# richox/orz

Hardware: AMD Instinct MI355X
Metric: orz -l1 encode throughput (enwik8-shaped text, 100 MB, one 16 MiB block in flight) (higher is better)
Workload: dtype u8

## Files before the change

### orz_amd/csrc/backend_hip.h

```cpp
#pragma once
#include <hip/hip_runtime.h>

#include <cxxabi.h>

#include <chrono>
#include <condition_variable>
#include <algorithm>
#include <atomic>
#include <cstring>
#include <map>
#include <mutex>
#include <rocprim/rocprim.hpp>
#include <stdexcept>
#include <string>
#include <type_traits>
#include <vector>

#include "orz_kernels.h"
#include "orz_parse.h"
#include "orz_symrank.h"

namespace orz {

#define ORZ_HIP_CHECK(expr)                                                                              \
// ... 527 lines not shown
        ORZ_HIP_CHECK(ce);
        hipGraphExec_t ex = nullptr;
        hipError_t e = hipGraphInstantiate(&ex, g, nullptr, nullptr, 0);
        (void)hipGraphDestroy(g);
        if (e != hipSuccess) throw std::runtime_error(std::string("hipGraphInstantiate: ") + hipGetErrorString(e));
        graph_exec_[key] = ex;
        ORZ_HIP_CHECK(hipGraphLaunch(ex, stream_));
    }
    void graph_capture_abort() {
        if (!capturing_) return;
        capturing_ = false;
        hipGraph_t g = nullptr;
        (void)hipStreamEndCapture(stream_, &g);
        stream_ = run_stream_;
        if (g) (void)hipGraphDestroy(g);
        (void)hipGetLastError();
    }
    void set_graphs(bool on) { graphs_ = on; }
    void clear_graphs() {
        for (auto& kv : graph_exec_) (void)hipGraphExecDestroy(kv.second);
        graph_exec_.clear();
    }
    void set_profile(bool on) { profile_ = on; nev_used_ = 0; nest_ = 0; }
    void begin_encode() { nev_used_ = 0; nest_ = 0; ev_used_ = 0; }
    bool profile() const { return profile_; }

    void symrank(uint16_t* srstate, const uint32_t* gsym, uint16_t* grank, const uint32_t* rstart, uint32_t nitems, uint32_t* flags,
                 uint16_t* backup, uint16_t* keep) {
        static_assert((512 * kSrWords * 2) % 8 == 0, "the tables are copied in 8-byte words");
        const uint32_t nw = 512 * kSrWords * 2 / 8;
        launch(nw, SymGuardBegin{reinterpret_cast<const uint64_t*>(srstate), reinterpret_cast<uint64_t*>(backup), nw, flags});
        Bracket br(*this, profile_ ? KernelNames::lib("orz_symrank_kernel (+ guard)") : 0);
        timed_begin(1);
        hipLaunchKernelGGL(orz_symrank_kernel, dim3(512), dim3(64), 0, stream_, srstate, gsym, grank, rstart, (const uint16_t*)nullptr,
                           (const uint32_t*)nullptr);
        ORZ_HIP_CHECK(hipGetLastError());
        timed_end(1);
        const char* inj = getenv("ORZ_SYMRANK_INJECT");
        const long inject = inj ? atol(inj) : -1;
        if (inject >= 0 && (uint32_t)inject < nitems) launch(1, SymInject{gsym, grank, (uint32_t)inject});
        launch(SymCheck::kThreads, SymCheck{gsym, grank, nitems, flags, nullptr});
        hipLaunchKernelGGL(orz_symrank_kernel, dim3(512), dim3(64), 0, stream_, srstate, gsym, grank, rstart, (const uint16_t*)backup,
                           (const uint32_t*)flags);
        ORZ_HIP_CHECK(hipGetLastError());
        launch(SymCheck::kThreads, SymCheck{gsym, grank, nitems, flags + 1, flags});
        static const bool verify = getenv("ORZ_SYMRANK_VERIFY") && atoi(getenv("ORZ_SYMRANK_VERIFY"));
        if (verify && keep) {
            launch(SymCompare::kThreads, SymKeep{grank, keep, nitems});
            hipLaunchKernelGGL(orz_symrank_kernel, dim3(512), dim3(64), 0, stream_, srstate, gsym, grank, rstart, (const uint16_t*)backup,
                               (const uint32_t*)nullptr);
            ORZ_HIP_CHECK(hipGetLastError());
            launch(SymCompare::kThreads, SymCompare{grank, keep, nitems, flags + 2});
        }
    }

   private:
    void* arena_take(size_t bytes) {
        if (!arena_on_) return nullptr;
        if (!arena_tried_) {
            arena_tried_ = true;
            const char* v = getenv("ORZ_ARENA_MB");
            const size_t mb = v ? (size_t)strtoull(v, nullptr, 10) : 0;
            if (mb) {
                (void)hipSetDevice(device_);
                void* p = nullptr;
                if (hipMalloc(&p, mb << 20) == hipSuccess) { arena_ = (char*)p; arena_bytes_ = mb << 20; }
                else (void)hipGetLastError();
            }
        }
        if (!arena_) return nullptr;
        const size_t align = bytes >= (1u << 20) ? (2u << 20) : 256;
        const size_t at = (arena_used_ + align - 1) / align * align;
        if (at + bytes > arena_bytes_) return nullptr;
        arena_used_ = at + bytes;
        arena_live_++;
        return arena_ + at;
    }
    char* arena_ = nullptr;
    size_t arena_bytes_ = 0, arena_used_ = 0, arena_live_ = 0;
    bool arena_tried_ = false, arena_on_ = false;
    int device_;
    bool lone_ = true, rank_prio_ = false;
// ... 25 lines not shown
```

### orz_amd/csrc/orz_capi.hip

```cpp
#include <cstdlib>
#include <cstring>
#include <map>
#include <memory>
#include <new>
#include <string>
#include <atomic>
#include <thread>
#include <vector>

#include "../../include/orz_hip.h"
#include "backend_hip.h"
#include "orz_decode_device.h"
#include "orz_decode_index.h"
#include "orz_decode_range.h"
#include "orz_decode_scatter.h"
#include "orz_host_decode.h"
#include "orz_planes.h"
#include "orz_decode_check.h"
#include "orz_stream.h"
#include "orz_fast_step.h"

namespace {
struct HwQueueDefault {
    HwQueueDefault() { setenv("GPU_MAX_HW_QUEUES", "16", 0); }
} g_hw_queue_default;


thread_local std::string g_err;
int fail(int code, const std::string& msg) {
    g_err = msg;
    return code;
}

orz::Cfg to_cfg(const orz_lzcfg* c) {
    return orz::Cfg{(int)c->match_depth, (int)c->lazy_match_depth1, (int)c->lazy_match_depth2};
}
// ... 30 lines not shown
    }
}

using Enc = orz::StreamEncoder<orz::HipBackend>;

bool mode_from_env() {
    const char* v = std::getenv("ORZ_MODE");
    return !(v && std::string(v) == "exact");
}

bool verify_decode_on() {
    const char* v = std::getenv("ORZ_VERIFY");
    return v && std::string(v) == "decode";
}
void verify_stream_decode(const uint8_t* src, size_t n, bool src_on_device, const uint8_t* out, size_t out_len) {
    std::vector<uint8_t> host;
    if (src_on_device && n) {
        host.resize(n);
        ORZ_HIP_CHECK(hipMemcpy(host.data(), src, n, hipMemcpyDeviceToHost));
        src = host.data();
    }
    orz::host::DecodeCheck chk;
    chk.feed_input(src, n);
    chk.feed_output(out, out_len);
    chk.finish();
}

unsigned window_for(const orz::HipBackend& be, const orz_lzcfg& c, unsigned asked) {
    if (asked) return asked;
    const size_t dmax = std::max(c.match_depth, std::max(c.lazy_match_depth1, c.lazy_match_depth2));
    return be.resident_parse_waves(orz::ParseLds::make((uint32_t)dmax, false).total);
}

}

struct orz_stream {
    std::unique_ptr<orz::HipBackend> be;
    std::unique_ptr<Enc> enc;
    orz_lzcfg cfg;
    unsigned seg, win;
    orz::ItemTrace trace;
    bool tracing = false;
    orz::FastTableCapture tables;
    bool fast = false;
    unsigned ftile = orz::kFastTile, frounds = orz::kFastRounds;
    unsigned unit = 0;
    double kernel_ms[4] = {0, 0, 0, 0};
    uint64_t kernel_n[4] = {0, 0, 0, 0};
    std::vector<orz::KernelRow> ktable;
    void rebuild() {
        std::unique_ptr<Enc> fresh;
        try {
            fresh.reset(new Enc(*be, to_cfg(&cfg), seg, fast ? 64 : window_for(*be, cfg, win), fast, ftile, frounds));
        } catch (const std::exception&) {
            if (!enc) throw;
            (void)hipGetLastError();
            enc.reset();
            be->clear_graphs();
            fresh.reset(new Enc(*be, to_cfg(&cfg), seg, fast ? 64 : window_for(*be, cfg, win), fast, ftile, frounds));
        }
        if (fast && unit && !getenv("ORZ_FAST_UNIT")) fresh->set_unit(unit);
        be->clear_graphs();
        enc = std::move(fresh);
        enc->trace = tracing ? &trace : nullptr;
        enc->tables = &tables;
    }
// ... 19 lines not shown
    std::unique_ptr<Enc> enc;
    orz_lzcfg cfg{0, 0, 0};
    unsigned seg, win;
    std::vector<uint8_t> framed;
    size_t framed_pos = 0;
    std::vector<size_t> chunk_end_spos;
    size_t next_chunk = 0;
    size_t expect_spos = 0;
    bool first_block = true;
    bool slid = false;
};

extern "C" {

const char* orz_last_error(void) { return g_err.c_str(); }
const char* orz_version(void) { return "orz_hip 0.1 (bitstream: richox/orz 1.6.1)"; }

int orz_device_count(void) {
    int n = 0;
    if (hipGetDeviceCount(&n) != hipSuccess) return 0;
    return n;
}

int orz_lzcfg_from_level(int level, orz_lzcfg* out) {
    if (!out) return fail(ORZ_EINVAL, "null cfg");
    switch (level) {
        case 0: *out = orz_lzcfg{5, 3, 2}; return ORZ_OK;
        case 1: *out = orz_lzcfg{15, 9, 6}; return ORZ_OK;
        case 2: *out = orz_lzcfg{45, 27, 18}; return ORZ_OK;
        default: return fail(ORZ_EINVAL, "invalid level");
    }
}

void orz_free(void* p) { std::free(p); }

static orz_stream* stream_new(int device, const orz_lzcfg* cfg, bool lone) {
    if (!cfg_ok(cfg)) { fail(ORZ_EINVAL, "bad LZCfg"); return nullptr; }
    try {
        if (device < 0 || device >= orz_device_count()) { fail(ORZ_ENODEV, "no such HIP device"); return nullptr; }
        std::unique_ptr<orz_stream> s(new orz_stream);
        s->be.reset(new orz::HipBackend(device, lone));
        s->be->enable_arena();
        s->cfg = *cfg;
        s->seg = env_u("ORZ_SEG", kDefaultSeg);
        s->win = env_u("ORZ_WIN", 0);
        s->fast = mode_from_env();
        s->ftile = env_u("ORZ_FAST_TILE", orz::kFastTile);
        s->frounds = env_u("ORZ_FAST_ROUNDS", orz::kFastRounds);
        s->be->set_graphs(env_u("ORZ_GRAPHS", 1) != 0);
        if (!lone) s->unit = orz::kNewMax;
        s->rebuild();
        return s.release();
    } catch (const std::exception& e) {
        fail(ORZ_ENODEV, e.what());
        return nullptr;
    }
}
orz_stream* orz_stream_new(int device, const orz_lzcfg* cfg) { return stream_new(device, cfg, true); }
void orz_stream_free(orz_stream* s) {
    if (!s) return;
    s->enc.reset();
    s->be.reset();
    delete s;
}
int orz_stream_set_tuning(orz_stream* s, unsigned seg_bytes, unsigned window_segs) {
    if (!s) return fail(ORZ_EINVAL, "null stream");
    try {
        s->reconfigure([&] {
            if (seg_bytes) s->seg = seg_bytes;
            if (window_segs) s->win = window_segs;
        });
        return ORZ_OK;
    } catch (const std::exception& e) {
        return fail(ORZ_EINVAL, e.what());
    }
}
int orz_stream_set_mode(orz_stream* s, int mode, unsigned tile_bytes, unsigned rounds) {
    if (!s || (mode != ORZ_MODE_EXACT && mode != ORZ_MODE_FAST)) return fail(ORZ_EINVAL, "bad mode");
    try {
        s->reconfigure([&] {
            s->fast = mode == ORZ_MODE_FAST;
            if (tile_bytes) s->ftile = tile_bytes;
            if (rounds) s->frounds = rounds;
        });
        return ORZ_OK;
    } catch (const std::exception& e) {
        return fail(ORZ_EINVAL, e.what());
    }
}
int orz_stream_set_profile(orz_stream* s, int on) {
    if (!s) return fail(ORZ_EINVAL, "null stream");
    s->be->set_profile(on != 0);
    return ORZ_OK;
}
int orz_stream_get_kernel_times(orz_stream* s, double* ms4, uint64_t* launches4) {
    if (!s || !ms4 || !launches4) return fail(ORZ_EINVAL, "null argument");
// ... 49 lines not shown
    } else {
        (void)hipGetLastError();
    }
    struct Disarm {
        orz::FastTableCapture& c;
        ~Disarm() { c.arm = -1; }
    } disarm{s->tables};
    struct ClearPatches {
        orz_stream* s;
        ~ClearPatches() { if (s->enc) s->enc->clear_item_patches(); }
    } clear_patches{s};
    const auto r = orz::encode_stream_device(*s->enc, be, (const uint8_t*)src, n, src_on_device != 0, d_dst, d_cap, pinned);
    if (stats) {
        float total = 0;
        ORZ_HIP_CHECK(hipEventElapsedTime(&total, ev.a, ev.b));
        const orz::EncodeStats& st = s->enc->stats;
        stats->blocks = st.blocks; stats->sweeps = st.sweeps; stats->seg_evals = st.seg_evals;
        stats->items = st.items; stats->chunks = st.chunks; stats->in_bytes = st.in_bytes;
        stats->out_bytes = r.len;
        stats->t_prep_s = st.t_prep; stats->t_parse_s = st.t_parse; stats->t_post_s = st.t_post;
        stats->parse_kernel_ms = be.collect_timed(&stats->parse_launches, s->kernel_ms, s->kernel_n);
        stats->total_ms = total;
        stats->host_syncs = st.host_syncs + be.take_host_syncs();
        if (be.profile()) s->ktable = be.collect_named();
    }
    return r;
}
int orz_stream_encode(orz_stream* s, const void* src, size_t n, int src_on_device, uint8_t** dst, size_t* dst_len,
                      orz_encode_stats* stats) {
    if (!s || !dst || !dst_len || (!src && n)) return fail(ORZ_EINVAL, "null argument");
    if (!s->enc) return fail(ORZ_ENOMEM, "the stream has no encoder (a reconfiguration ran out of device memory)");
    try {
        const auto r = stream_encode_device(s, src, n, src_on_device, nullptr, 0, stats);
        uint8_t* p = (uint8_t*)std::malloc(r.len ? r.len : 1);
        if (!p) return fail(ORZ_ENOMEM, "out of host memory");
        const hipError_t ce = hipMemcpy(p, r.data, r.len, hipMemcpyDeviceToHost);
        if (stats) stats->host_syncs += 1;
        if (ce != hipSuccess) { std::free(p); return fail(ORZ_ENODEV, hipGetErrorString(ce)); }
        if (verify_decode_on()) {
            try { verify_stream_decode((const uint8_t*)src, n, src_on_device != 0, p, r.len); } catch (...) { std::free(p); throw; }
        }
        *dst_len = r.len;
        *dst = p;
        return ORZ_OK;
    } catch (const std::bad_alloc&) {
        return fail(ORZ_ENOMEM, "out of host memory");
    } catch (const std::exception& e) {
        return fail(ORZ_ENODEV, e.what());
    }
}
size_t orz_stream_bound(size_t n) { return orz::stream_bound(n); }
int orz_stream_encode_to_device(orz_stream* s, const void* src, size_t n, int src_on_device, uint8_t* d_dst, size_t d_cap,
                                size_t* dst_len, orz_encode_stats* stats) {
    if (!s || !d_dst || !dst_len || (!src && n)) return fail(ORZ_EINVAL, "null argument");
    if (!s->enc) return fail(ORZ_ENOMEM, "the stream has no encoder (a reconfiguration ran out of device memory)");
    try {
        const auto r = stream_encode_device(s, src, n, src_on_device, d_dst, d_cap, stats);
        if (verify_decode_on()) {
            std::vector<uint8_t> host(r.len);
            ORZ_HIP_CHECK(hipMemcpy(host.data(), r.data, r.len, hipMemcpyDeviceToHost));
            verify_stream_decode((const uint8_t*)src, n, src_on_device != 0, host.data(), host.size());
        }
        *dst_len = r.len;
        return ORZ_OK;
    } catch (const std::bad_alloc&) {
        return fail(ORZ_ENOMEM, "out of host memory");
    } catch (const std::exception& e) {
        const std::string msg = e.what();
        return fail(msg.find("output buffer is too small") != std::string::npos ? ORZ_ENOMEM : ORZ_ENODEV, msg);
    }
}

int orz_stream_set_item_trace(orz_stream* s, int on) {
// ... 985 lines not shown
```

### orz_amd/csrc/orz_symrank.h

```cpp
#pragma once
#include "orz_kernels.h"

namespace orz {

#if defined(__HIPCC__)

constexpr uint32_t kSrGroup = 32;
constexpr uint32_t kSrPad = 448;
constexpr uint32_t kSrValOff = 0;
constexpr uint32_t kSrIdxOff = 896;
constexpr uint32_t kSrSnapOff = 1792;
constexpr uint32_t kSrLdsBytes = kSrSnapOff + kSrGroup * 128;

#define ORZ_SRL_WB_1 "s_waitcnt lgkmcnt(1)\n\tds_write_b16 %[aw], %[n]\n\t"
#define ORZ_SRL_WB_0 "s_nop 0\n\t"
#define ORZ_SRL_ITEM(P, J2, SNAP, PREV)                                                                                  \
    "ds_write_b16 %[l2], %[x] offset:" SNAP "\n\t"                                                                       \
    "v_readlane_b32 %[si], %[x], " J2 "\n\t"                                                                             \
    "s_cmpk_ge_u32 %[qw], 0x1860\n\t"                         \
    ORZ_SRL_WB_##PREV                                                                                                    \
    "v_mov_b32 %[vi], %[si]\n\t"                                                                                         \
    "s_cbranch_scc1 " P "30f\n\t"                                                                                        \
    P "31:\n\t"                                                                                                          \
    "s_add_u32 %[qw], %[qw], 16\n\t"                                                                                     \
    "s_add_u32 %[qa], %[qa], %[si]\n\t"                                                                                  \
    "s_sub_u32 %[qa], %[qa], %[qc]\n\t"                                                                                  \
    "s_cmp_ge_u32 %[qa], %[qw]\n\t"                                                                                      \
    "v_lshrrev_b32 %[t], 4, %[vi]\n\t"                                                                                   \
    "v_lshrrev_b32 %[h], 1, %[vi]\n\t"                                                                                   \
    "v_sub_u32 %[t], %[vi], %[t]\n\t"                                                                                    \
    "s_cbranch_scc1 " P "40f\n\t"                                                                                        \
    P "41:\n\t"                                                                                                          \
    "v_sub_u32_e64 %[t], %[t], %[q]\n\t"                                                                                 \
    "v_cmp_eq_u32_e64 %[m1], %[x], %[vi]\n\t"                                                                            \
    "v_max3_i32 %[nx], %[t], %[h], 0\n\t"                                   \
    "v_add_u32 %[y], %[vi], %[nx]\n\t"                                                                                   \
    "v_cmp_eq_u32_e64 %[m3], %[x], %[nx]\n\t"                                                                            \
    "v_lshrrev_b32 %[y], 1, %[y]\n\t"                            \
    "v_cndmask_b32_e64 %[rr], %[nx], %[y], %[m01]\n\t"                    \
    "v_cmp_eq_u32_e32 vcc, %[x], %[y]\n\t"                                                                               \
    "v_cndmask_b32_e64 %[rw], %[y], %[vi], %[m01]\n\t"                      \
    "v_lshl_add_u32 %[ar], %[rr], 1, %[base]\n\t"                                                                        \
    "v_cndmask_b32_e64 %[x], %[x], %[y], %[m3]\n\t"                                                   \
    "ds_read_u16 %[n], %[ar]\n\t"                                                                                        \
    "v_cndmask_b32_e32 %[x], %[x], %[vi], vcc\n\t"             \
    "v_lshl_add_u32 %[aw], %[rw], 1, %[base]\n\t"                                                                        \
    "v_cndmask_b32_e64 %[x], %[x], %[nx], %[m1]\n\t"
#define ORZ_SRL_WBS_1 "s_waitcnt lgkmcnt(1)\n\tds_write_b16 %[aw], %[n]\n\t"
#define ORZ_SRL_WBS_0 "s_nop 1\n\t"
#define ORZ_SRL_ITEM_S(J2, SNAP, PREV)                                                                                   \
    "ds_write_b16 %[l2], %[x] offset:" SNAP "\n\t"                                                                       \
    "v_readlane_b32 %[si], %[x], " J2 "\n\t"                                                                             \
    ORZ_SRL_WBS_##PREV                                                                                                   \
    "v_mov_b32 %[vi], %[si]\n\t"                                                                                         \
    "v_mad_i32_i24 %[t], %[vi], 15, %[c15]\n\t"  \
    "v_lshrrev_b32 %[h], 1, %[vi]\n\t"                                                                                   \
    "v_cmp_eq_u32_e64 %[m1], %[x], %[vi]\n\t"                                                                            \
    "v_ashrrev_i32 %[t], 4, %[t]\n\t"                                                                                    \
    "v_max3_i32 %[nx], %[t], %[h], 0\n\t"                                                                                \
    "v_add_u32 %[y], %[vi], %[nx]\n\t"                                                                                   \
    "v_cmp_eq_u32_e64 %[m3], %[x], %[nx]\n\t"                                                                            \
    "v_lshrrev_b32 %[y], 1, %[y]\n\t"                                                                                    \
    "v_cndmask_b32_e64 %[rr], %[nx], %[y], %[m01]\n\t"                                                                   \
    "v_cmp_eq_u32_e32 vcc, %[x], %[y]\n\t"                                                                               \
    "v_cndmask_b32_e64 %[rw], %[y], %[vi], %[m01]\n\t"                                                                   \
    "v_lshl_add_u32 %[ar], %[rr], 1, %[base]\n\t"                                                                        \
    "v_cndmask_b32_e64 %[x], %[x], %[y], %[m3]\n\t"                                                                      \
    "ds_read_u16 %[n], %[ar]\n\t"                                                                                        \
    "v_cndmask_b32_e32 %[x], %[x], %[vi], vcc\n\t"                                                                       \
    "v_lshl_add_u32 %[aw], %[rw], 1, %[base]\n\t"                                                                        \
    "v_cndmask_b32_e64 %[x], %[x], %[nx], %[m1]\n\t"
#define ORZ_SRL_SIDE(P)                                                                                                  \
    P "30:\n\t"                                                             \
    "s_lshr_b32 %[s0], %[qw], 4\n\t"                                                                                     \
    "s_mul_i32 %[s1], %[s0], %[qc]\n\t"                                                                                  \
    "s_add_u32 %[s1], %[s1], %[qa]\n\t"                                                                                  \
    "s_mul_i32 %[s0], %[s0], 9\n\t"                                                                                      \
    "s_mul_hi_u32 %[s0], %[s0], 0xcccccccd\n\t"                                                                          \
    "s_lshr_b32 %[s0], %[s0], 3\n\t"                                                                                     \
    "s_mul_i32 %[s1], %[s1], 9\n\t"                                                                                      \
    "s_mul_hi_u32 %[s1], %[s1], 0xcccccccd\n\t"                                                                          \
    "s_lshr_b32 %[s1], %[s1], 3\n\t"                                                                                     \
    "s_lshl_b32 %[qw], %[s0], 4\n\t"                                                                                     \
    "s_mul_i32 %[s0], %[s0], %[qc]\n\t"                                                                                  \
    "s_sub_u32 %[qa], %[s1], %[s0]\n\t"                                                                                  \
    "s_branch " P "31b\n\t"                                                                                              \
    P "40:\n\t"                                                \
    "s_cmp_lt_i32 %[qa], 0\n\t"                                                                                          \
    "s_cbranch_scc1 " P "42f\n\t"                                                                                        \
    "s_sub_u32 %[qa], %[qa], %[qw]\n\t"                                                                                  \
    "s_add_u32 %[q], %[q], 1\n\t"                                                                                        \
    "s_add_u32 %[qc], %[qc], 16\n\t"                                                                                     \
    "s_branch " P "43f\n\t"                                                                                              \
    P "42:\n\t"                                                                                                          \
    "s_add_u32 %[qa], %[qa], %[qw]\n\t"                                                                                  \
    "s_sub_u32 %[q], %[q], 1\n\t"                                                                                        \
    "s_sub_u32 %[qc], %[qc], 16\n\t"                                                                                     \
    P "43:\n\t"                                                                                                          \
    "s_cmp_ge_u32 %[qa], %[qw]\n\t"                                                                                      \
    "s_cbranch_scc1 " P "40b\n\t"                                                                                        \
    "s_branch " P "41b\n\t"

// ... 35 lines not shown
    ORZ_SRL_SIDE("101") \
    ORZ_SRL_SIDE("102") \
    ORZ_SRL_SIDE("103") \
    ORZ_SRL_SIDE("104") \
    ORZ_SRL_SIDE("105") \
    ORZ_SRL_SIDE("106") \
    ORZ_SRL_SIDE("107") \
    ORZ_SRL_SIDE("108") \
    ORZ_SRL_SIDE("109") \
    ORZ_SRL_SIDE("110") \
    ORZ_SRL_SIDE("111") \
    ORZ_SRL_SIDE("112") \
    ORZ_SRL_SIDE("113") \
    ORZ_SRL_SIDE("114") \
    ORZ_SRL_SIDE("115") \
    ORZ_SRL_SIDE("116") \
    ORZ_SRL_SIDE("117") \
    ORZ_SRL_SIDE("118") \
    ORZ_SRL_SIDE("119") \
    ORZ_SRL_SIDE("120") \
    ORZ_SRL_SIDE("121") \
    ORZ_SRL_SIDE("122") \
    ORZ_SRL_SIDE("123") \
    ORZ_SRL_SIDE("124") \
    ORZ_SRL_SIDE("125") \
    ORZ_SRL_SIDE("126") \
    ORZ_SRL_SIDE("127") \
    ORZ_SRL_SIDE("128") \
    ORZ_SRL_SIDE("129") \
    ORZ_SRL_SIDE("130") \
    ORZ_SRL_SIDE("131") \
    "9:\n\t"

#define ORZ_SRL_GROUP_S \
    ORZ_SRL_ITEM_S("0", "0", 0) \
    ORZ_SRL_ITEM_S("2", "128", 1) \
    ORZ_SRL_ITEM_S("4", "256", 1) \
    ORZ_SRL_ITEM_S("6", "384", 1) \
    ORZ_SRL_ITEM_S("8", "512", 1) \
    ORZ_SRL_ITEM_S("10", "640", 1) \
    ORZ_SRL_ITEM_S("12", "768", 1) \
    ORZ_SRL_ITEM_S("14", "896", 1) \
    ORZ_SRL_ITEM_S("16", "1024", 1) \
    ORZ_SRL_ITEM_S("18", "1152", 1) \
    ORZ_SRL_ITEM_S("20", "1280", 1) \
    ORZ_SRL_ITEM_S("22", "1408", 1) \
    ORZ_SRL_ITEM_S("24", "1536", 1) \
    ORZ_SRL_ITEM_S("26", "1664", 1) \
    ORZ_SRL_ITEM_S("28", "1792", 1) \
    ORZ_SRL_ITEM_S("30", "1920", 1) \
    ORZ_SRL_ITEM_S("32", "2048", 1) \
    ORZ_SRL_ITEM_S("34", "2176", 1) \
    ORZ_SRL_ITEM_S("36", "2304", 1) \
    ORZ_SRL_ITEM_S("38", "2432", 1) \
    ORZ_SRL_ITEM_S("40", "2560", 1) \
    ORZ_SRL_ITEM_S("42", "2688", 1) \
    ORZ_SRL_ITEM_S("44", "2816", 1) \
    ORZ_SRL_ITEM_S("46", "2944", 1) \
    ORZ_SRL_ITEM_S("48", "3072", 1) \
    ORZ_SRL_ITEM_S("50", "3200", 1) \
    ORZ_SRL_ITEM_S("52", "3328", 1) \
    ORZ_SRL_ITEM_S("54", "3456", 1) \
    ORZ_SRL_ITEM_S("56", "3584", 1) \
    ORZ_SRL_ITEM_S("58", "3712", 1) \
    ORZ_SRL_ITEM_S("60", "3840", 1) \
    ORZ_SRL_ITEM_S("62", "3968", 1)

__global__ __launch_bounds__(64) void orz_symrank_kernel(uint16_t* srstate, const uint32_t* gsym, uint16_t* grank,
                                                         const uint32_t* rstart, const uint16_t* state_in, const uint32_t* only_if) {
    __shared__ __attribute__((aligned(16))) uint16_t lds[kSrLdsBytes / 2];
    uint16_t* const val = lds + kSrValOff / 2;
    uint16_t* const idx = lds + kSrIdxOff / 2;
    const uint32_t c = blockIdx.x, lane = threadIdx.x;
    if (only_if && *only_if == 0) return;
    const uint32_t a = rstart[c], e = rstart[c + 1];
    if (a >= e) return;
    __builtin_amdgcn_s_setprio(3);
    uint16_t* state = srstate + (size_t)c * kSrWords;
    const uint16_t* sin = state_in ? state_in + (size_t)c * kSrWords : state;
    const uint32_t base = (uint32_t)(uintptr_t)lds;
    auto slot_of = [&](uint32_t sym) -> uint32_t { return base + kSrIdxOff + 2 * sym; };
    auto sym_of = [&](uint32_t slot) -> uint32_t { return (slot - base - kSrIdxOff) >> 1; };
    typedef __attribute__((address_space(3))) uint16_t lds_u16;
    auto at = [&](uint32_t slot) -> lds_u16& { return *reinterpret_cast<lds_u16*>((uintptr_t)slot); };
    for (uint32_t i = lane; i < kSrPad; i += 64) {
        val[i] = (uint16_t)slot_of(i < kSyms ? sin[i] : i);
        idx[i] = i < kSyms ? sin[kSyms + i] : (uint16_t)i;
    }
    uint32_t cnt = __builtin_amdgcn_readfirstlane((int)(sin[2 * kSyms] | ((uint32_t)sin[2 * kSyms + 1] << 16)));
    uint32_t sum = __builtin_amdgcn_readfirstlane((int)(sin[2 * kSyms + 2] | ((uint32_t)sin[2 * kSyms + 3] << 16)));
    __syncthreads();
    bool idx_ok = true;
    auto rebuild_idx = [&]() {
        uint32_t s[7];
#pragma unroll
        for (uint32_t m = 0; m < 7; m++) s[m] = val[lane + 64 * m];
#pragma unroll
        for (uint32_t m = 0; m < 7; m++) at(s[m]) = (uint16_t)(lane + 64 * m);
    };
    auto load_pairs = [&](uint32_t j0) -> uint32_t {
        return j0 + kSrGroup <= e ? gsym[j0 + (lane >> 1)] : 0u;
    };
    auto out_rank = [&](uint32_t ri, uint32_t ru) -> uint16_t { return (uint16_t)(ri == ru ? kSyms - 1 : ri - (ri > ru)); };
    const uint32_t l2 = base + kSrSnapOff + 2 * lane;
    const uint32_t* const snap_pair = reinterpret_cast<const uint32_t*>(lds + kSrSnapOff / 2 + (lane & 31) * 66);
    const uint64_t m01 = 1;
    uint32_t j = a;
    while (j < e) {
        if (cnt >= 192 && e - j >= kSrGroup) {
            uint32_t q = (uint32_t)__builtin_amdgcn_readfirstlane((int)((sum >> 4) / cnt));
            uint32_t pairs = load_pairs(j);
            do {
                uint32_t s[7];
#pragma unroll
                for (uint32_t m = 0; m < 7; m++) s[m] = val[lane + 64 * m];
#pragma unroll
                for (uint32_t m = 0; m < 7; m++) at(s[m]) = (uint16_t)(lane + 64 * m);
                const uint32_t symslot = slot_of((lane & 1) ? pairs >> 16 : pairs & 0xffff);
                const int x0 = (int)at(symslot);
                pairs = load_pairs(j + kSrGroup);
                q = (uint32_t)__builtin_amdgcn_readfirstlane((int)q);
                uint32_t si;
                uint64_t m1, m3;
                int x, vi, t, h, nx, y, rr, rw, ar, aw, n;
                bool done = false;
                if (cnt >= 327 && q < 32) {
                    x = x0;
                    asm volatile("s_waitcnt lgkmcnt(0)\n\t"
                                 ORZ_SRL_GROUP_S
                                 "s_waitcnt lgkmcnt(0)\n\tds_write_b16 %[aw], %[n]\n\t"
                                 "v_lshl_add_u32 %[ar], %[x], 1, %[base]\n\tds_write_b16 %[ar], %[sym]\n\t"
                                 : [x] "+v"(x), [si] "=&s"(si), [m1] "=&s"(m1), [m3] "=&s"(m3), [vi] "=&v"(vi), [t] "=&v"(t), [h] "=&v"(h),
                                   [nx] "=&v"(nx), [y] "=&v"(y), [rr] "=&v"(rr), [rw] "=&v"(rw), [ar] "=&v"(ar), [aw] "=&v"(aw), [n] "=&v"(n)
                                 : [l2] "v"(l2), [base] "s"(base), [sym] "v"(symslot), [m01] "s"(m01), [c15] "s"(15 - (int)(q << 4))
                                 : "vcc", "memory");
                    const uint32_t two = *snap_pair;
                    uint32_t ps = lane < kSrGroup ? two & 0xffff : 0;
                    ps += (uint32_t)__builtin_amdgcn_update_dpp(0, (int)ps, 0x111, 0xf, 0xf, true);
                    ps += (uint32_t)__builtin_amdgcn_update_dpp(0, (int)ps, 0x112, 0xf, 0xf, true);
                    ps += (uint32_t)__builtin_amdgcn_update_dpp(0, (int)ps, 0x114, 0xf, 0xf, true);
                    ps += (uint32_t)__builtin_amdgcn_update_dpp(0, (int)ps, 0x118, 0xf, 0xf, true);
                    ps += (uint32_t)__builtin_amdgcn_update_dpp(0, (int)ps, 0x142, 0xa, 0xf, true);
                    const uint32_t r = kSyms + 1 - cnt;
                    const uint32_t pr = r > 0 && r < kSrGroup ? (uint32_t)__builtin_amdgcn_readlane((int)ps, (int)((r - 1) & 31)) : 0u;
                    const uint32_t scaled = (sum + pr) * 9 / 10;
                    const bool after = lane >= r;
                    const uint32_t cnt_k = after ? (kSyms + 1) * 9 / 10 + (lane - r) + 1 : cnt + lane + 1;
                    const uint32_t sum_k = after ? scaled + (ps - pr) : sum + ps;
                    const uint32_t lo = (q << 4) * cnt_k;
                    const bool ok = sum_k >= lo && sum_k - lo < (cnt_k << 4);
                    if (__ballot(lane < kSrGroup && !ok) == 0) {
                        if (lane < kSrGroup) grank[j + lane] = out_rank(two & 0xffff, two >> 16);
                        cnt = (uint32_t)__builtin_amdgcn_readlane((int)cnt_k, 31);
                        sum = (uint32_t)__builtin_amdgcn_readlane((int)sum_k, 31);
                        done = true;
                    } else {
#pragma unroll
                        for (uint32_t m = 0; m < 7; m++) val[lane + 64 * m] = (uint16_t)s[m];
                    }
                }
                if (!done) {
                    uint32_t s0, s1;
                    uint32_t qw = (uint32_t)__builtin_amdgcn_readfirstlane((int)(cnt << 4));
                    uint32_t qc = (uint32_t)__builtin_amdgcn_readfirstlane((int)(q << 4));
                    uint32_t qa = (uint32_t)__builtin_amdgcn_readfirstlane((int)(sum - q * qw));
                    x = x0;
                    asm volatile("s_waitcnt lgkmcnt(0)\n\t"
                                 ORZ_SRL_GROUP
                                 "s_waitcnt lgkmcnt(0)\n\tds_write_b16 %[aw], %[n]\n\t"
                                 "v_lshl_add_u32 %[ar], %[x], 1, %[base]\n\tds_write_b16 %[ar], %[sym]\n\t"
                                 : [x] "+v"(x), [qw] "+s"(qw), [qa] "+s"(qa), [qc] "+s"(qc), [q] "+s"(q), [si] "=&s"(si), [s0] "=&s"(s0),
                                   [s1] "=&s"(s1), [m1] "=&s"(m1), [m3] "=&s"(m3), [vi] "=&v"(vi), [t] "=&v"(t), [h] "=&v"(h), [nx] "=&v"(nx),
                                   [y] "=&v"(y), [rr] "=&v"(rr), [rw] "=&v"(rw), [ar] "=&v"(ar), [aw] "=&v"(aw), [n] "=&v"(n)
                                 : [l2] "v"(l2), [base] "s"(base), [sym] "v"(symslot), [m01] "s"(m01)
                                 : "scc", "vcc", "memory");
                    cnt = qw >> 4;
                    sum = qa + q * qw;
                    const uint32_t two = *snap_pair;
                    if (lane < kSrGroup) grank[j + lane] = out_rank(two & 0xffff, two >> 16);
                }
                j += kSrGroup;
            } while (e - j >= kSrGroup);
            idx_ok = false;
            continue;
        }
        if (!idx_ok) { rebuild_idx(); idx_ok = true; }
        const uint32_t g = __builtin_amdgcn_readfirstlane((int)gsym[j]);
        const uint32_t v = g & 0xffff, vun = g >> 16;
        const uint32_t i = idx[v], iu = idx[vun];
        if (cnt > kSyms) {
            cnt = cnt * 9 / 10;
            sum = sum * 9 / 10;
        }
        cnt += 1;
        sum += i;
        const uint32_t dec = ((i >> 4) + (((sum >> 4) / cnt) & 0xffff)) & 0xffff, half = i >> 1;
        uint32_t nx = i > dec ? i - dec : 0;
        nx = nx > half ? nx : half;
        const uint32_t y = (i + nx) >> 1;
        const uint32_t nv1 = val[y], nv2 = val[nx];
        val[y] = (uint16_t)nv2; at(nv2) = (uint16_t)y;
        val[i] = (uint16_t)nv1; at(nv1) = (uint16_t)i;
        val[nx] = (uint16_t)slot_of(v); idx[v] = (uint16_t)nx;
        if (lane == 0) grank[j] = out_rank(i, iu);
        j += 1;
    }
    if (!idx_ok) rebuild_idx();
    __syncthreads();
    for (uint32_t i = lane; i < kSyms; i += 64) { state[i] = (uint16_t)sym_of(val[i]); state[kSyms + i] = idx[i]; }
    if (lane == 0) {
        state[2 * kSyms] = (uint16_t)cnt;
        state[2 * kSyms + 1] = (uint16_t)(cnt >> 16);
        state[2 * kSyms + 2] = (uint16_t)sum;
        state[2 * kSyms + 3] = (uint16_t)(sum >> 16);
    }
}

#endif

}
```

Baseline: 495.6.

## Split symrank into producer and LDS-update helper waves; pool pinned result buffers

The symrank kernel now launches two waves per block. Wave 0 computes the rank chain and publishes snapshots, while wave 1 applies the LDS swap writes in sub-batches, synchronised by s_barrier and a control word in LDS. The intent is to take the serial read-modify-write LDS traffic off the critical wave. Separately, encode results of 1 MiB or more are copied into pooled pinned host buffers with an async copy, avoiding the cost of staging through pageable memory. The risks are barrier overhead per sub-batch, subtle ordering bugs in the hand-written asm protocol, and pooled buffers outliving their stream handles.

```diff
diff --git a/orz_amd/csrc/backend_hip.h b/orz_amd/csrc/backend_hip.h
--- a/orz_amd/csrc/backend_hip.h
+++ b/orz_amd/csrc/backend_hip.h
@@ -583,7 +583,7 @@
         launch(nw, SymGuardBegin{reinterpret_cast<const uint64_t*>(srstate), reinterpret_cast<uint64_t*>(backup), nw, flags});
         Bracket br(*this, profile_ ? KernelNames::lib("orz_symrank_kernel (+ guard)") : 0);
         timed_begin(1);
-        hipLaunchKernelGGL(orz_symrank_kernel, dim3(512), dim3(64), 0, stream_, srstate, gsym, grank, rstart, (const uint16_t*)nullptr,
+        hipLaunchKernelGGL(orz_symrank_kernel, dim3(512), dim3(kSrThreads), 0, stream_, srstate, gsym, grank, rstart, (const uint16_t*)nullptr,
                            (const uint32_t*)nullptr);
         ORZ_HIP_CHECK(hipGetLastError());
         timed_end(1);
@@ -591,14 +591,14 @@
         const long inject = inj ? atol(inj) : -1;
         if (inject >= 0 && (uint32_t)inject < nitems) launch(1, SymInject{gsym, grank, (uint32_t)inject});
         launch(SymCheck::kThreads, SymCheck{gsym, grank, nitems, flags, nullptr});
-        hipLaunchKernelGGL(orz_symrank_kernel, dim3(512), dim3(64), 0, stream_, srstate, gsym, grank, rstart, (const uint16_t*)backup,
+        hipLaunchKernelGGL(orz_symrank_kernel, dim3(512), dim3(kSrThreads), 0, stream_, srstate, gsym, grank, rstart, (const uint16_t*)backup,
                            (const uint32_t*)flags);
         ORZ_HIP_CHECK(hipGetLastError());
         launch(SymCheck::kThreads, SymCheck{gsym, grank, nitems, flags + 1, flags});
         static const bool verify = getenv("ORZ_SYMRANK_VERIFY") && atoi(getenv("ORZ_SYMRANK_VERIFY"));
         if (verify && keep) {
             launch(SymCompare::kThreads, SymKeep{grank, keep, nitems});
-            hipLaunchKernelGGL(orz_symrank_kernel, dim3(512), dim3(64), 0, stream_, srstate, gsym, grank, rstart, (const uint16_t*)backup,
+            hipLaunchKernelGGL(orz_symrank_kernel, dim3(512), dim3(kSrThreads), 0, stream_, srstate, gsym, grank, rstart, (const uint16_t*)backup,
                                (const uint32_t*)nullptr);
             ORZ_HIP_CHECK(hipGetLastError());
             launch(SymCompare::kThreads, SymCompare{grank, keep, nitems, flags + 2});
diff --git a/orz_amd/csrc/orz_capi.hip b/orz_amd/csrc/orz_capi.hip
--- a/orz_amd/csrc/orz_capi.hip
+++ b/orz_amd/csrc/orz_capi.hip
@@ -2,6 +2,7 @@
 #include <cstring>
 #include <map>
 #include <memory>
+#include <mutex>
 #include <new>
 #include <string>
 #include <atomic>
@@ -98,6 +99,77 @@
     return be.resident_parse_waves(orz::ParseLds::make((uint32_t)dmax, false).total);
 }
 
+}
+
+namespace {
+constexpr size_t kPoolMin = size_t(1) << 20;
+constexpr size_t kPoolIdleMax = 2;
+struct ResultPool {
+    std::mutex mu;
+    std::map<void*, size_t> out;
+    std::vector<std::pair<void*, size_t>> idle;
+    size_t handles = 0;
+    static size_t capacity_for(size_t n) {
+        size_t c = kPoolMin;
+        while (c < n) c <<= 1;
+        return c;
+    }
+    void* take(size_t n) {
+        const size_t cap = capacity_for(n);
+        {
+            std::lock_guard<std::mutex> g(mu);
+            size_t best = idle.size();
+            for (size_t i = 0; i < idle.size(); i++)
+                if (idle[i].second >= cap && (best == idle.size() || idle[i].second < idle[best].second)) best = i;
+            if (best < idle.size()) {
+                void* p = idle[best].first;
+                out[p] = idle[best].second;
+                idle.erase(idle.begin() + (long)best);
+                return p;
+            }
+        }
+        void* p = nullptr;
+        if (hipHostMalloc(&p, cap, hipHostMallocPortable) != hipSuccess || !p) {
+            (void)hipGetLastError();
+            return nullptr;
+        }
+        std::lock_guard<std::mutex> g(mu);
+        out[p] = cap;
+        return p;
+    }
+    bool give(void* p) {
+        size_t cap = 0;
+        {
+            std::lock_guard<std::mutex> g(mu);
+            auto it = out.find(p);
+            if (it == out.end()) return false;
+            cap = it->second;
+            out.erase(it);
+            if (handles > 0 && idle.size() < kPoolIdleMax) {
+                idle.emplace_back(p, cap);
+                return true;
+            }
+        }
+        (void)hipHostFree(p);
+        return true;
+    }
+    void handle_born() {
+        std::lock_guard<std::mutex> g(mu);
+        handles++;
+    }
+    void handle_gone() {
+        std::vector<std::pair<void*, size_t>> drop;
+        {
+            std::lock_guard<std::mutex> g(mu);
+            if (handles > 0 && --handles == 0) drop.swap(idle);
+        }
+        for (auto& b : drop) (void)hipHostFree(b.first);
+    }
+};
+ResultPool& result_pool() {
+    static ResultPool* const pool = new ResultPool;
+    return *pool;
+}
 }
 
 struct orz_stream {
@@ -183,7 +255,10 @@
     }
 }
 
-void orz_free(void* p) { std::free(p); }
+void orz_free(void* p) {
+    if (!p) return;
+    if (!result_pool().give(p)) std::free(p);
+}
 
 static orz_stream* stream_new(int device, const orz_lzcfg* cfg, bool lone) {
     if (!cfg_ok(cfg)) { fail(ORZ_EINVAL, "bad LZCfg"); return nullptr; }
@@ -201,6 +276,7 @@
         s->be->set_graphs(env_u("ORZ_GRAPHS", 1) != 0);
         if (!lone) s->unit = orz::kNewMax;
         s->rebuild();
+        result_pool().handle_born();
         return s.release();
     } catch (const std::exception& e) {
         fail(ORZ_ENODEV, e.what());
@@ -213,6 +289,7 @@
     s->enc.reset();
     s->be.reset();
     delete s;
+    result_pool().handle_gone();
 }
 int orz_stream_set_tuning(orz_stream* s, unsigned seg_bytes, unsigned window_segs) {
     if (!s) return fail(ORZ_EINVAL, "null stream");
@@ -328,13 +405,15 @@
     if (!s->enc) return fail(ORZ_ENOMEM, "the stream has no encoder (a reconfiguration ran out of device memory)");
     try {
         const auto r = stream_encode_device(s, src, n, src_on_device, nullptr, 0, stats);
-        uint8_t* p = (uint8_t*)std::malloc(r.len ? r.len : 1);
+        uint8_t* p = r.len >= kPoolMin ? (uint8_t*)result_pool().take(r.len) : nullptr;
+        if (!p) p = (uint8_t*)std::malloc(r.len ? r.len : 1);
         if (!p) return fail(ORZ_ENOMEM, "out of host memory");
-        const hipError_t ce = hipMemcpy(p, r.data, r.len, hipMemcpyDeviceToHost);
+        hipError_t ce = hipMemcpyAsync(p, r.data, r.len, hipMemcpyDeviceToHost, s->be->stream());
+        if (ce == hipSuccess) ce = hipStreamSynchronize(s->be->stream());
         if (stats) stats->host_syncs += 1;
-        if (ce != hipSuccess) { std::free(p); return fail(ORZ_ENODEV, hipGetErrorString(ce)); }
+        if (ce != hipSuccess) { orz_free(p); return fail(ORZ_ENODEV, hipGetErrorString(ce)); }
         if (verify_decode_on()) {
-            try { verify_stream_decode((const uint8_t*)src, n, src_on_device != 0, p, r.len); } catch (...) { std::free(p); throw; }
+            try { verify_stream_decode((const uint8_t*)src, n, src_on_device != 0, p, r.len); } catch (...) { orz_free(p); throw; }
         }
         *dst_len = r.len;
         *dst = p;
diff --git a/orz_amd/csrc/orz_symrank.h b/orz_amd/csrc/orz_symrank.h
--- a/orz_amd/csrc/orz_symrank.h
+++ b/orz_amd/csrc/orz_symrank.h
@@ -10,7 +10,15 @@
 constexpr uint32_t kSrValOff = 0;
 constexpr uint32_t kSrIdxOff = 896;
 constexpr uint32_t kSrSnapOff = 1792;
-constexpr uint32_t kSrLdsBytes = kSrSnapOff + kSrGroup * 128;
+constexpr uint32_t kSrCtlOff = kSrSnapOff + kSrGroup * 128;
+constexpr uint32_t kSrLdsBytes = kSrCtlOff + 16;
+constexpr uint32_t kSrThreads = 128;
+#ifndef ORZ_SR_SUB
+#define ORZ_SR_SUB 8
+#endif
+constexpr uint32_t kSrSub = ORZ_SR_SUB;
+static_assert(kSrSub == 4 || kSrSub == 8, "a sub-batch is 4 or 8 items");
+constexpr uint32_t kSrCtlExit = 0;
 
 #define ORZ_SRL_WB_1 "s_waitcnt lgkmcnt(1)\n\tds_write_b16 %[aw], %[n]\n\t"
 #define ORZ_SRL_WB_0 "s_nop 0\n\t"
@@ -44,30 +52,6 @@
     "v_cndmask_b32_e64 %[x], %[x], %[y], %[m3]\n\t"                                                   \
     "ds_read_u16 %[n], %[ar]\n\t"                                                                                        \
     "v_cndmask_b32_e32 %[x], %[x], %[vi], vcc\n\t"             \
-    "v_lshl_add_u32 %[aw], %[rw], 1, %[base]\n\t"                                                                        \
-    "v_cndmask_b32_e64 %[x], %[x], %[nx], %[m1]\n\t"
-#define ORZ_SRL_WBS_1 "s_waitcnt lgkmcnt(1)\n\tds_write_b16 %[aw], %[n]\n\t"
-#define ORZ_SRL_WBS_0 "s_nop 1\n\t"
-#define ORZ_SRL_ITEM_S(J2, SNAP, PREV)                                                                                   \
-    "ds_write_b16 %[l2], %[x] offset:" SNAP "\n\t"                                                                       \
-    "v_readlane_b32 %[si], %[x], " J2 "\n\t"                                                                             \
-    ORZ_SRL_WBS_##PREV                                                                                                   \
-    "v_mov_b32 %[vi], %[si]\n\t"                                                                                         \
-    "v_mad_i32_i24 %[t], %[vi], 15, %[c15]\n\t"  \
-    "v_lshrrev_b32 %[h], 1, %[vi]\n\t"                                                                                   \
-    "v_cmp_eq_u32_e64 %[m1], %[x], %[vi]\n\t"                                                                            \
-    "v_ashrrev_i32 %[t], 4, %[t]\n\t"                                                                                    \
-    "v_max3_i32 %[nx], %[t], %[h], 0\n\t"                                                                                \
-    "v_add_u32 %[y], %[vi], %[nx]\n\t"                                                                                   \
-    "v_cmp_eq_u32_e64 %[m3], %[x], %[nx]\n\t"                                                                            \
-    "v_lshrrev_b32 %[y], 1, %[y]\n\t"                                                                                    \
-    "v_cndmask_b32_e64 %[rr], %[nx], %[y], %[m01]\n\t"                                                                   \
-    "v_cmp_eq_u32_e32 vcc, %[x], %[y]\n\t"                                                                               \
-    "v_cndmask_b32_e64 %[rw], %[y], %[vi], %[m01]\n\t"                                                                   \
-    "v_lshl_add_u32 %[ar], %[rr], 1, %[base]\n\t"                                                                        \
-    "v_cndmask_b32_e64 %[x], %[x], %[y], %[m3]\n\t"                                                                      \
-    "ds_read_u16 %[n], %[ar]\n\t"                                                                                        \
-    "v_cndmask_b32_e32 %[x], %[x], %[vi], vcc\n\t"                                                                       \
     "v_lshl_add_u32 %[aw], %[rw], 1, %[base]\n\t"                                                                        \
     "v_cndmask_b32_e64 %[x], %[x], %[nx], %[m1]\n\t"
 #define ORZ_SRL_SIDE(P)                                                                                                  \
@@ -169,46 +153,85 @@
     ORZ_SRL_SIDE("131") \
     "9:\n\t"
 
-#define ORZ_SRL_GROUP_S \
-    ORZ_SRL_ITEM_S("0", "0", 0) \
-    ORZ_SRL_ITEM_S("2", "128", 1) \
-    ORZ_SRL_ITEM_S("4", "256", 1) \
-    ORZ_SRL_ITEM_S("6", "384", 1) \
-    ORZ_SRL_ITEM_S("8", "512", 1) \
-    ORZ_SRL_ITEM_S("10", "640", 1) \
-    ORZ_SRL_ITEM_S("12", "768", 1) \
-    ORZ_SRL_ITEM_S("14", "896", 1) \
-    ORZ_SRL_ITEM_S("16", "1024", 1) \
-    ORZ_SRL_ITEM_S("18", "1152", 1) \
-    ORZ_SRL_ITEM_S("20", "1280", 1) \
-    ORZ_SRL_ITEM_S("22", "1408", 1) \
-    ORZ_SRL_ITEM_S("24", "1536", 1) \
-    ORZ_SRL_ITEM_S("26", "1664", 1) \
-    ORZ_SRL_ITEM_S("28", "1792", 1) \
-    ORZ_SRL_ITEM_S("30", "1920", 1) \
-    ORZ_SRL_ITEM_S("32", "2048", 1) \
-    ORZ_SRL_ITEM_S("34", "2176", 1) \
-    ORZ_SRL_ITEM_S("36", "2304", 1) \
-    ORZ_SRL_ITEM_S("38", "2432", 1) \
-    ORZ_SRL_ITEM_S("40", "2560", 1) \
-    ORZ_SRL_ITEM_S("42", "2688", 1) \
-    ORZ_SRL_ITEM_S("44", "2816", 1) \
-    ORZ_SRL_ITEM_S("46", "2944", 1) \
-    ORZ_SRL_ITEM_S("48", "3072", 1) \
-    ORZ_SRL_ITEM_S("50", "3200", 1) \
-    ORZ_SRL_ITEM_S("52", "3328", 1) \
-    ORZ_SRL_ITEM_S("54", "3456", 1) \
-    ORZ_SRL_ITEM_S("56", "3584", 1) \
-    ORZ_SRL_ITEM_S("58", "3712", 1) \
-    ORZ_SRL_ITEM_S("60", "3840", 1) \
-    ORZ_SRL_ITEM_S("62", "3968", 1)
-
-__global__ __launch_bounds__(64) void orz_symrank_kernel(uint16_t* srstate, const uint32_t* gsym, uint16_t* grank,
-                                                         const uint32_t* rstart, const uint16_t* state_in, const uint32_t* only_if) {
+#define ORZ_SRT_ITEM(J2, SNAP)                                                                                           \
+    "ds_write_b16 %[l2], %[x] offset:" SNAP "\n\t"                                                                       \
+    "v_readlane_b32 %[si], %[x], " J2 "\n\t"                                                                             \
+    "s_nop 1\n\t"                                                                                                        \
+    "v_mov_b32 %[vi], %[si]\n\t"                                                                                         \
+    "v_mad_i32_i24 %[t], %[vi], 15, %[c15]\n\t"                                                                          \
+    "v_lshrrev_b32 %[h], 1, %[vi]\n\t"                                                                                   \
+    "v_ashrrev_i32 %[t], 4, %[t]\n\t"                                                                                    \
+    "v_max3_i32 %[nx], %[t], %[h], 0\n\t"                                                                                \
+    "v_add_u32 %[y], %[vi], %[nx]\n\t"                                                                                   \
+    "v_cmp_eq_u32_e64 %[m3], %[x], %[nx]\n\t"                                                                            \
+    "v_lshrrev_b32 %[y], 1, %[y]\n\t"                                                                                    \
+    "v_cmp_eq_u32_e32 vcc, %[x], %[y]\n\t"                                                                               \
+    "v_cmp_eq_u32_e64 %[m1], %[x], %[vi]\n\t"                                                                            \
+    "v_cndmask_b32_e64 %[x], %[x], %[y], %[m3]\n\t"                                                   \
+    "v_cndmask_b32_e32 %[x], %[x], %[vi], vcc\n\t"                                                         \
+    "v_cndmask_b32_e64 %[x], %[x], %[nx], %[m1]\n\t"
+#define ORZ_SRT_SYNC "s_waitcnt lgkmcnt(0)\n\ts_barrier\n\t"
+#if ORZ_SR_SUB == 4
+#define ORZ_SRT_SYNC4 ORZ_SRT_SYNC
+#else
+#define ORZ_SRT_SYNC4
+#endif
+#define ORZ_SRT_GROUP \
+    ORZ_SRT_ITEM("0", "0") \
+    ORZ_SRT_ITEM("2", "128") \
+    ORZ_SRT_ITEM("4", "256") \
+    ORZ_SRT_ITEM("6", "384") \
+    ORZ_SRT_SYNC4 \
+    ORZ_SRT_ITEM("8", "512") \
+    ORZ_SRT_ITEM("10", "640") \
+    ORZ_SRT_ITEM("12", "768") \
+    ORZ_SRT_ITEM("14", "896") \
+    ORZ_SRT_SYNC \
+    ORZ_SRT_ITEM("16", "1024") \
+    ORZ_SRT_ITEM("18", "1152") \
+    ORZ_SRT_ITEM("20", "1280") \
+    ORZ_SRT_ITEM("22", "1408") \
+    ORZ_SRT_SYNC4 \
+    ORZ_SRT_ITEM("24", "1536") \
+    ORZ_SRT_ITEM("26", "1664") \
+    ORZ_SRT_ITEM("28", "1792") \
+    ORZ_SRT_ITEM("30", "1920") \
+    ORZ_SRT_SYNC \
+    ORZ_SRT_ITEM("32", "2048") \
+    ORZ_SRT_ITEM("34", "2176") \
+    ORZ_SRT_ITEM("36", "2304") \
+    ORZ_SRT_ITEM("38", "2432") \
+    ORZ_SRT_SYNC4 \
+    ORZ_SRT_ITEM("40", "2560") \
+    ORZ_SRT_ITEM("42", "2688") \
+    ORZ_SRT_ITEM("44", "2816") \
+    ORZ_SRT_ITEM("46", "2944") \
+    ORZ_SRT_SYNC \
+    ORZ_SRT_ITEM("48", "3072") \
+    ORZ_SRT_ITEM("50", "3200") \
+    ORZ_SRT_ITEM("52", "3328") \
+    ORZ_SRT_ITEM("54", "3456") \
+    ORZ_SRT_SYNC4 \
+    ORZ_SRT_ITEM("56", "3584") \
+    ORZ_SRT_ITEM("58", "3712") \
+    ORZ_SRT_ITEM("60", "3840") \
+    ORZ_SRT_ITEM("62", "3968") \
+    ORZ_SRT_SYNC
+
+#define ORZ_SRU_ITEM "ds_read_u16 %[n], %[ar]\n\ts_waitcnt lgkmcnt(0)\n\tds_write_b16 %[aw], %[n]\n\ts_lshl_b64 exec, exec, 2\n\t"
+#if ORZ_SR_SUB == 4
+#define ORZ_SRU_BATCH ORZ_SRU_ITEM ORZ_SRU_ITEM ORZ_SRU_ITEM ORZ_SRU_ITEM
+#else
+#define ORZ_SRU_BATCH ORZ_SRU_ITEM ORZ_SRU_ITEM ORZ_SRU_ITEM ORZ_SRU_ITEM ORZ_SRU_ITEM ORZ_SRU_ITEM ORZ_SRU_ITEM ORZ_SRU_ITEM
+#endif
+
+__global__ __launch_bounds__(kSrThreads) void orz_symrank_kernel(uint16_t* srstate, const uint32_t* gsym, uint16_t* grank,
+                                                                 const uint32_t* rstart, const uint16_t* state_in, const uint32_t* only_if) {
     __shared__ __attribute__((aligned(16))) uint16_t lds[kSrLdsBytes / 2];
     uint16_t* const val = lds + kSrValOff / 2;
     uint16_t* const idx = lds + kSrIdxOff / 2;
-    const uint32_t c = blockIdx.x, lane = threadIdx.x;
+    const uint32_t c = blockIdx.x, tid = threadIdx.x, lane = tid & 63;
+    const uint32_t wave = (uint32_t)__builtin_amdgcn_readfirstlane((int)(tid >> 6));
     if (only_if && *only_if == 0) return;
     const uint32_t a = rstart[c], e = rstart[c + 1];
     if (a >= e) return;
@@ -219,14 +242,43 @@
     auto slot_of = [&](uint32_t sym) -> uint32_t { return base + kSrIdxOff + 2 * sym; };
     auto sym_of = [&](uint32_t slot) -> uint32_t { return (slot - base - kSrIdxOff) >> 1; };
     typedef __attribute__((address_space(3))) uint16_t lds_u16;
+    typedef __attribute__((address_space(3))) volatile uint32_t lds_word;
+    lds_word& ctl = *reinterpret_cast<lds_word*>((uintptr_t)(base + kSrCtlOff));
     auto at = [&](uint32_t slot) -> lds_u16& { return *reinterpret_cast<lds_u16*>((uintptr_t)slot); };
-    for (uint32_t i = lane; i < kSrPad; i += 64) {
+    for (uint32_t i = tid; i < kSrPad; i += kSrThreads) {
         val[i] = (uint16_t)slot_of(i < kSyms ? sin[i] : i);
         idx[i] = i < kSyms ? sin[kSyms + i] : (uint16_t)i;
     }
     uint32_t cnt = __builtin_amdgcn_readfirstlane((int)(sin[2 * kSyms] | ((uint32_t)sin[2 * kSyms + 1] << 16)));
     uint32_t sum = __builtin_amdgcn_readfirstlane((int)(sin[2 * kSyms + 2] | ((uint32_t)sin[2 * kSyms + 3] << 16)));
     __syncthreads();
+    if (wave == 1) {
+        for (;;) {
+            asm volatile("s_barrier" ::: "memory");
+            const uint32_t w = (uint32_t)__builtin_amdgcn_readfirstlane((int)ctl);
+            if (w == kSrCtlExit) break;
+            const int c15 = (int)w - 1024;
+#pragma unroll 1
+            for (uint32_t b = 0; b < kSrGroup / kSrSub; b++) {
+                if (b) asm volatile("s_barrier" ::: "memory");
+                const uint32_t k = b * kSrSub + ((lane >> 1) & (kSrSub - 1));
+                const int i = (int)at(base + kSrSnapOff + k * 132);
+                const int t = (i * 15 + c15) >> 4, h = i >> 1;
+                const int nx = t > h ? t : h;
+                const int y = (i + nx) >> 1;
+                const uint32_t ar = base + 2 * (uint32_t)((lane & 1) ? nx : y), aw = base + 2 * (uint32_t)((lane & 1) ? y : i);
+                uint64_t sv;
+                int n;
+                asm volatile("s_mov_b64 %[sv], exec\n\ts_mov_b64 exec, 3\n\t"
+                             ORZ_SRU_BATCH
+                             "s_mov_b64 exec, %[sv]\n\t"
+                             : [sv] "=&s"(sv), [n] "=&v"(n)
+                             : [ar] "v"(ar), [aw] "v"(aw)
+                             : "scc", "memory");
+            }
+            asm volatile("s_waitcnt lgkmcnt(0)\n\ts_barrier" ::: "memory");
+        }
+    }
     bool idx_ok = true;
     auto rebuild_idx = [&]() {
         uint32_t s[7];
@@ -242,7 +294,7 @@
     const uint32_t l2 = base + kSrSnapOff + 2 * lane;
     const uint32_t* const snap_pair = reinterpret_cast<const uint32_t*>(lds + kSrSnapOff / 2 + (lane & 31) * 66);
     const uint64_t m01 = 1;
-    uint32_t j = a;
+    uint32_t j = wave == 0 ? a : e;
     while (j < e) {
         if (cnt >= 192 && e - j >= kSrGroup) {
             uint32_t q = (uint32_t)__builtin_amdgcn_readfirstlane((int)((sum >> 4) / cnt));
@@ -262,14 +314,14 @@
                 int x, vi, t, h, nx, y, rr, rw, ar, aw, n;
                 bool done = false;
                 if (cnt >= 327 && q < 32) {
+                    const int c15 = 15 - (int)(q << 4);
+                    ctl = (uint32_t)(1024 + c15);
                     x = x0;
                     asm volatile("s_waitcnt lgkmcnt(0)\n\t"
-                                 ORZ_SRL_GROUP_S
-                                 "s_waitcnt lgkmcnt(0)\n\tds_write_b16 %[aw], %[n]\n\t"
-                                 "v_lshl_add_u32 %[ar], %[x], 1, %[base]\n\tds_write_b16 %[ar], %[sym]\n\t"
+                                 ORZ_SRT_GROUP
                                  : [x] "+v"(x), [si] "=&s"(si), [m1] "=&s"(m1), [m3] "=&s"(m3), [vi] "=&v"(vi), [t] "=&v"(t), [h] "=&v"(h),
-                                   [nx] "=&v"(nx), [y] "=&v"(y), [rr] "=&v"(rr), [rw] "=&v"(rw), [ar] "=&v"(ar), [aw] "=&v"(aw), [n] "=&v"(n)
-                                 : [l2] "v"(l2), [base] "s"(base), [sym] "v"(symslot), [m01] "s"(m01), [c15] "s"(15 - (int)(q << 4))
+                                   [nx] "=&v"(nx), [y] "=&v"(y)
+                                 : [l2] "v"(l2), [c15] "s"(c15)
                                  : "vcc", "memory");
                     const uint32_t two = *snap_pair;
                     uint32_t ps = lane < kSrGroup ? two & 0xffff : 0;
@@ -286,10 +338,15 @@
                     const uint32_t sum_k = after ? scaled + (ps - pr) : sum + ps;
                     const uint32_t lo = (q << 4) * cnt_k;
                     const bool ok = sum_k >= lo && sum_k - lo < (cnt_k << 4);
-                    if (__ballot(lane < kSrGroup && !ok) == 0) {
+                    const bool pass = __ballot(lane < kSrGroup && !ok) == 0;
+                    if (pass) {
                         if (lane < kSrGroup) grank[j + lane] = out_rank(two & 0xffff, two >> 16);
                         cnt = (uint32_t)__builtin_amdgcn_readlane((int)cnt_k, 31);
                         sum = (uint32_t)__builtin_amdgcn_readlane((int)sum_k, 31);
+                    }
+                    asm volatile("s_waitcnt lgkmcnt(0)\n\ts_barrier" ::: "memory");
+                    if (pass) {
+                        val[x] = (uint16_t)symslot;
                         done = true;
                     } else {
 #pragma unroll
@@ -342,10 +399,13 @@
         if (lane == 0) grank[j] = out_rank(i, iu);
         j += 1;
     }
-    if (!idx_ok) rebuild_idx();
-    __syncthreads();
-    for (uint32_t i = lane; i < kSyms; i += 64) { state[i] = (uint16_t)sym_of(val[i]); state[kSyms + i] = idx[i]; }
-    if (lane == 0) {
+    if (wave == 0) {
+        if (!idx_ok) rebuild_idx();
+        ctl = kSrCtlExit;
+        asm volatile("s_waitcnt lgkmcnt(0)\n\ts_barrier" ::: "memory");
+    }
+    for (uint32_t i = tid; i < kSyms; i += kSrThreads) { state[i] = (uint16_t)sym_of(val[i]); state[kSyms + i] = idx[i]; }
+    if (tid == 0) {
         state[2 * kSyms] = (uint16_t)cnt;
         state[2 * kSyms + 1] = (uint16_t)(cnt >> 16);
         state[2 * kSyms + 2] = (uint16_t)sum;
```

Result: faster. 535.3, median of 6 (+8.0%).
